# qdrant/qdrant

Measured on AMD Instinct MI355X. Metric: QPS @ recall@10, brute-force, d=768 10M vecs, f32 cosine top-10, higher is better.
Workload: dtype f32 (int8 prefilter + exact f32 re-score)

## Files before the change

### qdrant_amd/csrc/api_core.hip

```cpp
#include "api_internal.hpp"

namespace qmx {

static thread_local std::string g_last_error;
const std::string &last_error_text() { return g_last_error; }

void set_error(const char *fmt, ...) {
    char buf[1024];
    va_list ap;
    va_start(ap, fmt);
    vsnprintf(buf, sizeof(buf), fmt, ap);
    va_end(ap);
    g_last_error = buf;
}

int32_t hip_status(hipError_t e, const char *what, const char *file, int line) {
    set_error("HIP error %d (%s) at %s:%d: %s", (int)e, hipGetErrorString(e), file, line, what);
    (void)hipGetLastError();
    switch (e) {
        case hipErrorOutOfMemory: return QMX_ERR_OUT_OF_MEMORY;
        case hipErrorNoDevice:
        case hipErrorInvalidDevice:
        case hipErrorNoBinaryForGpu:
        case hipErrorInsufficientDriver: return QMX_ERR_NO_DEVICE;
        case hipErrorNotReady: return QMX_ERR_NOT_READY;
        case hipErrorInvalidValue: return QMX_ERR_BAD_ARG;
        default: return QMX_ERR_OTHER;
    }
}

static const char *const g_option_names[OPT_COUNT] = {"no_mfma_scan", "no_mfma16", "no_prescan", "prescan_shift", "hnsw_log_cap", "no_split_scan", "split_min_queries", "no_split256", "no_pq_pair", "no_pq_prefilter", "pq_prefilter_min_queries", "hnsw_pq_per_cu", "tq_rotate_block", "no_topk_small", "verify_max_per_query", "hnsw_pq_direct_walk", "hnsw_pq_table_build", "hnsw_no_pq_prefilter", "hnsw_no_lds_visited", "pq_lut_no_lds", "hnsw_per_cu", "hnsw_reference_heap_order", "tq_wide_min_queries", "tq_wide_high_digit", "sq_wide_min_queries", "i8_resident", "i8_dense_epilogue", "i8_sample_stride", "i8_sample_scan", "i8_sample_rows", "prescan_beside_scan", "group_matrix_bytes", "debug"};
struct OptionTable {
    std::atomic<int64_t> v[OPT_COUNT];
    int64_t initial[OPT_COUNT];
    OptionTable() {
        for (int i = 0; i < OPT_COUNT; ++i) {
            char env[64] = "QMX_";
            size_t k = 4;
            for (const char *c = g_option_names[i]; *c && k + 1 < sizeof(env); ++c) env[k++] = (char)toupper((unsigned char)*c);
            env[k] = 0;
            const char *e = getenv(env);
            int64_t val = 0;
            if (e) { val = (*e >= '0' && *e <= '9') ? atoll(e) : 1; }
            if (i == OPT_PRESCAN_SHIFT && !e) val = 10;
            if (i == OPT_SPLIT_MIN_QUERIES && !e) val = 1;
            if (i == OPT_PQ_PREFILTER_MIN_QUERIES && !e) val = 4;
            if (i == OPT_TQ_WIDE_MIN_QUERIES && !e) val = 33;
            if (i == OPT_SQ_WIDE_MIN_QUERIES && !e) val = 33;
            if (i == OPT_I8_RESIDENT && !e) val = 1;
            if (i == OPT_I8_DENSE_EPILOGUE && !e) val = 1;
            if (i == OPT_I8_SAMPLE_STRIDE && !e) val = 16;
            if (i == OPT_I8_SAMPLE_SCAN && !e) val = 1;
            if (i == OPT_PRESCAN_BESIDE_SCAN && !e) val = 1;
            initial[i] = val;
            v[i].store(val, std::memory_order_relaxed);
        }
    }
};
static OptionTable g_options;
int64_t option(Option o) { return g_options.v[o].load(std::memory_order_relaxed); }

static thread_local const void *g_last_kernel = nullptr;
const void *last_noted_kernel() { return g_last_kernel; }
void note_kernel(const void *host_function) { g_last_kernel = host_function; }

void clear_stale_error() {
    hipError_t e = hipGetLastError();
    if (e != hipSuccess) {
// ... 98 lines not shown
```

### qdrant_amd/csrc/api_search.hip

```cpp
#include "api_internal.hpp"

extern "C" {

struct SearchCall {
    qmx_query *q;
    uint32_t top;
    const uint32_t *d_ids;
    uint64_t n_cand;
    qmx_scored_point *d_out;
    uint32_t *d_counts;
    const volatile uint8_t *is_stopped;
    qmx_counters *counters;
    bool timed;
    uint32_t launches;
};

static ScanArgs tile_args(const qmx_query *q, uint32_t top, uint64_t n_cand, uint32_t tile0, uint32_t nq_tile) {
    ScanArgs a;
    fill_args(q, tile0, nq_tile, a);
    a.n_cand = n_cand;
    a.top = top;
    return a;
}
static ScanArgs tile_args(const SearchCall &c, uint32_t tile0, uint32_t nq_tile) { return tile_args(c.q, c.top, c.n_cand, tile0, nq_tile); }
// ... 170 lines not shown
        ScanArgs a = tile_args(c, 0, nq_sub);
        a.queries = (const char *)q->sp_fq.p + (size_t)p0 * q->q_stride;
        if (fof_packed) a.del.filter_of = fof_packed + p0;
        a.partial = (uint64_t *)q->partial.p;
        a.gthr = gthr_packed + p0;
        a.run_if = run_if;
        const int fqt = (int)std::max<uint32_t>(16, pow2_ceil(nq_sub));
        a.partial_qt = (uint32_t)fqt;
        uint32_t grid = (uint32_t)q->seg->num_cus * 8;
        QMX_TRY(scan(q->stream, fqt, a, q->seg->num_cus, &grid));
        QMX_TRY(launch_merge_keys(q->stream, (const uint64_t *)q->partial.p, grid, (uint32_t)fqt, nq_sub, c.top, c.d_out, c.d_counts, c.top, 0, nullptr, run_if,
                                  ovf_list + p0));
        if (launches) *launches += 2;
    }
    return split_stage(q, "fallback (conditional)");
}

static int32_t pq_overflow_pass(const SearchCall &c, const SplitPlanLayout &pl) {
    qmx_query *q = c.q;
    const qmx_segment *s = q->seg;
    unsigned char *plan = (unsigned char *)q->sp_plan.p;
    uint32_t *ovf_list = (uint32_t *)(plan + pl.list);
    QMX_TRY(launch_split_plan(q->stream, (const uint32_t *)(plan + pl.ovf_q), q->nq, (const uint64_t *)q->gthr.p, ovf_list, (uint64_t *)(plan + pl.gthr_packed),
                              pl.list_cap, (uint32_t *)(plan + pl.count), (int *)(plan + pl.run16), (int *)(plan + pl.run64), pl.n_run64, (SplitStats *)plan, nullptr, 0,
                              nullptr));
    ScanArgs a = tile_args(c, 0, q->nq);
    a.q_map = ovf_list;
    a.run_if = (const int *)(plan + pl.count);
    const uint64_t want = (c.n_cand + 1023) / 1024, cap = std::max<uint64_t>(1, ((uint64_t)s->num_cus * 2 + q->nq - 1) / q->nq);
    uint32_t slabs = (uint32_t)std::max<uint64_t>(1, std::min(want, cap));
// ... 134 lines not shown
    QMX_TRY(verify_and_sort(c, vp, q->nq));
    QMX_TRY(overflow_passes(c, pl, q->nq, TQW_FQT, sq ? overflow_scan_sq : overflow_scan_tq, &c.launches));
    q->last_split = true;
    q->last_pq = false;
    q->last_fqt = TQW_FQT;
    close_counters(c, (uint64_t)q->nq * c.n_cand,
                   (uint64_t)n_tiles * c.n_cand * s->row_bytes + (uint64_t)((q->nq + MAX_QT_MFMA - 1) / MAX_QT_MFMA) * S * s->row_bytes, c.launches, q->nq);
    return QMX_OK;
}

struct SplitTiles {
    SplitPlanLayout pl;
    VerifyPool vp{};
    uint64_t S = 0;
    bool i8_sample = false;
    std::vector<std::pair<uint32_t, uint32_t>> tiles;
    SplitTiles(uint32_t nq, uint32_t fqt) : pl(nq, fqt) {}
};

static inline float split_rel_band(bool half, uint32_t dim) {
    const float acc = (float)dim * 1.1920929e-7f;
    return (half ? 9.765625e-4f + 9.5367432e-7f : 1.9073486e-6f) + acc;
}

static int32_t split_begin(const SearchCall &c, const SearchPlan &plan, SplitTiles &sp) {
    qmx_query *q = c.q;
    const qmx_segment *s = q->seg;
    QMX_TRY(q->sp_bq.reserve(split_query_bytes(s->dim)));
    QMX_TRY(q->sp_f32.reserve(SplitF32::floats * sizeof(float)));
    QMX_TRY(q->sp_cand.reserve((size_t)plan.split_qt * SPLIT_CAND_CAP * sizeof(uint64_t)));
// ... 92 lines not shown
    if (!sp.i8_sample) QMX_TRY(bound_enqueue(c, tile0, nq_tile, (const uint32_t *)q->sp_sample.p, sp.S, c.top, a.del, nullptr, true));
    QMX_TRY(split_stage(q, "prescan"));
    int *tile_ovf = (int *)((unsigned char *)q->sp_plan.p + sp.pl.tile_ovf) + sp.tiles.size();
    if (plan.route == ROUTE_I8_COPY) QMX_TRY(i8_copy_scan(c, sp, a, tile0, nq_tile, tile_ovf));
    else QMX_TRY(f16_split_scan(c, sp, a, tile0, nq_tile, tile_ovf));
    QMX_TRY(split_stage(q, "select"));
    sp.tiles.push_back({tile0, nq_tile});
    return QMX_OK;
}

static int32_t split_finish(const SearchCall &c, const SearchPlan &plan, const SplitTiles &sp) {
    qmx_query *q = c.q;
    const uint32_t first = sp.tiles.front().first, last = sp.tiles.back().first + sp.tiles.back().second;
    QMX_REQUIRE(first == 0, QMX_ERR_OTHER, "split tiles must start at query 0");
    QMX_TRY(verify_and_sort(c, sp.vp, last));
    QMX_TRY(overflow_passes(c, sp.pl, last, plan.split_fqt, overflow_scan_f32, nullptr));
    q->last_split = true;
    q->last_pq = false;
    q->last_fqt = plan.split_fqt;
    return QMX_OK;
}

static int32_t exact_tile(SearchCall &c, const SearchPlan &plan, uint32_t tile0, uint32_t nq_tile) {
    qmx_query *q = c.q;
    const qmx_segment *s = q->seg;
    const int qt = (int)pow2_ceil(nq_tile);
    for (uint32_t pass = 0; pass < plan.n_pass; ++pass) {
        QMX_CHECK_CANCELLED(c.is_stopped);
        const uint32_t off = pass * MAX_TOP_FAST;
        const uint32_t ptop = std::min<uint32_t>(MAX_TOP_FAST, c.top - off);
        ScanArgs a = tile_args(c, tile0, nq_tile);
        a.ids = c.d_ids;
        a.top = ptop;
        a.partial = (uint64_t *)q->partial.p;
// ... 25 lines not shown
    const qmx_segment *s = q->seg;
    if (is_sparse(s)) QMX_REFUSE_FILTERS(q);
    if (is_sparse(s)) return sparse_search_enqueue(q, top, d_ids, n_ids, d_out, d_counts, is_stopped, counters, timed);
    SearchCall c{q, top, d_ids, d_ids ? n_ids : s->scan_rows(), d_out, d_counts, is_stopped, counters, timed, 0};
    const SearchPlan plan = search_plan(q, top, d_ids, c.n_cand);
    q->last_counters = qmx_counters{};
    q->last_split = false;
    if (plan.route == ROUTE_TQ_L1) return tq_l1_search(c, plan);
    if (plan.route == ROUTE_PQ_PREFILTER) return pq_prefilter_search(c);
    if (plan.route == ROUTE_TQ_WIDE || plan.route == ROUTE_SQ_WIDE) return wide_exact_search(c);
    const uint32_t TQ = plan.tile_q;
    QMX_TRY(q->partial.reserve((size_t)s->num_cus * 8 * std::min<uint32_t>(TQ, MAX_QT_TOPK) * std::min<uint32_t>(top, MAX_TOP_FAST) * sizeof(uint64_t)));
    if (plan.n_pass > 1) QMX_TRY(q->bounds.reserve((size_t)TQ * sizeof(uint64_t)));
    QMX_TRY(q->gthr.reserve((size_t)std::max<uint32_t>(q->nq_padded, SPLIT_QT_MAX) * sizeof(uint64_t)));
    SplitTiles sp(q->nq, plan.split_fqt);
    if (plan.split()) QMX_TRY(split_begin(c, plan, sp));
    for (uint32_t tile0 = 0; tile0 < q->nq; tile0 += TQ) {
        const uint32_t nq_tile = std::min<uint32_t>(TQ, q->nq - tile0);
        if (plan.tile_splits(nq_tile)) QMX_TRY(split_tile(c, plan, sp, tile0, nq_tile));
        else QMX_TRY(exact_tile(c, plan, tile0, nq_tile));
    }
    if (!sp.tiles.empty()) QMX_TRY(split_finish(c, plan, sp));
    uint32_t split_q = 0;
    uint64_t bytes = 0;
    for (auto &t : sp.tiles) {
        split_q += t.second;
        bytes += c.n_cand * (uint64_t)s->dim * (s->split_i8 ? 1 : s->d_rows_split && s->split_half ? 2 : 4);
        if (sp.i8_sample) {
            const uint32_t group = split_i8_sample_queries(s->dim, t.second);
            bytes += (uint64_t)((t.second + group - 1) / group) * q->sp_sample_n * s->dim + (uint64_t)t.second * std::min<uint32_t>(top, MAX_TOP_FAST) * s->row_bytes;
// ... 217 lines not shown
```

### qdrant_amd/csrc/common.hpp

```cpp
#pragma once
#include <hip/hip_runtime.h>
#include <hip/hip_fp16.h>
#include <stdint.h>
#include <atomic>
#include <string>

#include "../../include/qdrant_amd.h"

namespace qmx {

void set_error(const char *fmt, ...);
int32_t hip_status(hipError_t e, const char *what, const char *file, int line);
void clear_stale_error();

enum Option {
    OPT_NO_MFMA_SCAN = 0,
    OPT_NO_MFMA16,
    OPT_NO_PRESCAN,
    OPT_PRESCAN_SHIFT,
    OPT_HNSW_LOG_CAP,
    OPT_NO_SPLIT_SCAN,
    OPT_SPLIT_MIN_QUERIES,
    OPT_NO_SPLIT256,
    OPT_NO_PQ_PAIR,
// ... 7 lines not shown
    OPT_HNSW_PQ_TABLE_BUILD,
    OPT_HNSW_NO_PQ_PREFILTER,
    OPT_HNSW_NO_LDS_VISITED,
    OPT_PQ_LUT_NO_LDS,
    OPT_HNSW_PER_CU,
    OPT_HNSW_REFERENCE_HEAP_ORDER,
    OPT_TQ_WIDE_MIN_QUERIES,
    OPT_TQ_WIDE_HIGH_DIGIT,
    OPT_SQ_WIDE_MIN_QUERIES,
    OPT_I8_RESIDENT,
    OPT_I8_DENSE_EPILOGUE,
    OPT_I8_SAMPLE_STRIDE,
    OPT_I8_SAMPLE_SCAN,
    OPT_I8_SAMPLE_ROWS,
    OPT_PRESCAN_BESIDE_SCAN,
    OPT_GROUP_MATRIX_BYTES,
    OPT_DEBUG,
    OPT_COUNT
};
int64_t option(Option o);
struct DeviceOnce {
    std::atomic<uint64_t> done{0};
    int dev = 0;
    bool need() {
        if (hipGetDevice(&dev) != hipSuccess) { dev = 0; return true; }
        return dev >= 64 || !(done.load(std::memory_order_acquire) & (1ull << dev));
    }
    void mark() { if (dev < 64) done.fetch_or(1ull << dev, std::memory_order_release); }
};
void note_kernel(const void *host_function);
// ... 123 lines not shown
```

### qdrant_amd/csrc/kernels.hpp

```cpp
#pragma once
#include "common.hpp"

namespace qmx {

constexpr int MAX_QT = 16;
constexpr int SCAN_BLOCK = 512;
constexpr int MAX_TOP_FAST = 64;

struct TqEc {
    const int16_t *weights;
    const float *xm;
    float weight_scale, mm_const;
};
struct ScanArgs {
    const void *rows;
    uint64_t n_rows;
    uint64_t row_stride;
    uint32_t dim;
    uint32_t nseg;
    uint32_t rem_pieces;
    uint32_t tail_start;
    uint32_t aux_off;
    uint32_t nq;
    const void *queries;
// ... 243 lines not shown
int32_t launch_scan_sq(hipStream_t st, int distance, int qt, ScanMode mode, const ScanArgs &a, int num_cus,
                       uint32_t *grid_out);
int32_t launch_sq_encode(hipStream_t st, int distance, const qmx_sq_params &sp, uint32_t dim, const float *in, uint64_t n,
                         uint8_t *codes_out, uint64_t codes_stride, float *offsets_out, uint8_t *rows_out, int is_query,
                         uint32_t aux_off);
int32_t launch_sq_split(hipStream_t st, const void *rows, uint64_t row_stride, uint64_t n, uint32_t actual_dim, void *codes,
                        float *offsets);
int32_t launch_sq_gather_rows(hipStream_t st, const void *codes, const float *offsets, uint32_t actual_dim, const uint32_t *ids,
                              uint32_t n, uint64_t n_rows, void *rows_out, int *err_flag);
int32_t launch_sq_internal_query(hipStream_t st, const void *codes, const float *offsets, uint32_t actual_dim, const uint32_t *ids,
                                 uint32_t nq, uint64_t n_rows, float shift, void *tile, uint32_t q_stride, uint32_t aux_off,
                                 int *err_flag);
bool mfma16_dim_ok(int qt, uint32_t dim);
bool mfma16_scan_ok(int qt, ScanMode mode, const ScanArgs &a);
int32_t launch_scan_f32_mfma16(hipStream_t st, int qt, const ScanArgs &a, int num_cus, uint32_t *grid_out);
bool split_scan_ok(const ScanArgs &a);
size_t split_query_bytes(uint32_t dim);
float split_row_scale(float row_maxabs);
int32_t launch_split_row_stats(hipStream_t st, const void *rows, uint64_t row_stride, uint64_t n, uint32_t dim, uint32_t *d_stats);
int32_t launch_split_pack_queries(hipStream_t st, const float *d_q, uint32_t nq, uint32_t dim, float *d_qmax, float *d_qnorm, void *d_bq, int half, uint32_t qt);
int32_t launch_split_thresholds(hipStream_t st, const uint64_t *d_gthr, const float *d_qnorm, const float *d_qmax, uint32_t nq, float rel_band, float row_norm_max,
                                float row_scale, float *d_scales, float *d_thr, float *d_band, uint32_t qt, uint32_t *d_cand_cnt, uint32_t n_cnt);
int32_t launch_scan_f32_split(hipStream_t st, const ScanArgs &a, const void *d_bq, float row_scale, const float *d_scales, const float *d_thr,
                              uint64_t *d_cand, uint32_t *d_cand_cnt, uint32_t cap, int num_cus, const void *d_rows_split, int half, void *d_wlists, uint32_t phase, uint32_t qt);
int32_t launch_regroup_lists(hipStream_t st, const DeletedView &del, const void *d_wlist, const uint32_t *d_wcnt, uint32_t wcap, uint32_t n_lists, uint64_t *d_cand,
                             uint32_t *d_cand_cnt, uint32_t cap, int *d_overflow);
size_t pq_rot_bytes(uint64_t n, uint32_t m);
bool pq_prefilter_shape_ok(uint32_t m, uint32_t ncent);
int32_t launch_pq_rotate(hipStream_t st, const void *codes, uint64_t row_stride, uint64_t n, uint32_t m, void *d_out);
size_t pq_prefilter_table_bytes(uint32_t m, uint32_t nq);
// ... 25 lines not shown
int32_t launch_split_select(hipStream_t st, const uint64_t *d_cand, const uint32_t *d_cand_cnt, uint32_t cap, const float *d_band, uint32_t nq, uint32_t top,
                            const VerifyPool &pool, uint32_t q_base, const int *d_tile_overflow, uint32_t *d_ovf_q, SplitStats *d_stats,
                            const float *d_t_exact = nullptr, bool tighten = false);
bool split_i8_dim_ok(uint32_t dim);
size_t split_i8_copy_bytes(uint64_t n, uint32_t dim);
size_t split_i8_query_bytes(uint32_t dim);
uint32_t split_i8_probe();
int32_t launch_split_i8_colstats(hipStream_t st, const void *rows, uint64_t row_stride, uint64_t n, uint32_t dim, uint32_t *d_colmax, float *d_colsq);
float split_i8_choose_scales(const float *colmax, const float *colsq, uint64_t n, uint32_t dim, float *scale);
int32_t launch_split_i8_rowstats(hipStream_t st, const void *rows, uint64_t row_stride, uint64_t n, uint32_t dim, const float *d_scale, uint32_t *d_stats);
int32_t launch_split_i8_copy(hipStream_t st, const void *rows, uint64_t row_stride, uint64_t n, uint32_t dim, const float *d_scale, void *d_out);
int32_t launch_split_i8_pack(hipStream_t st, const float *d_q, uint32_t nq, uint32_t dim, const float *d_scale, const uint64_t *d_gthr, const uint32_t *d_row_stats,
                             float row_norm_max, void *d_bq, float *d_qscale, float *d_band, float *d_thr, float *d_t_exact, uint32_t *d_cand_cnt, uint32_t n_cnt);
int32_t launch_scan_i8copy(hipStream_t st, const ScanArgs &a, const void *d_bq, const float *d_qscale, const float *d_thr, int num_cus, const void *d_rows_i8,
                           void *d_wlists, uint32_t phase);
int32_t launch_split_i8_probe(hipStream_t st, const uint64_t *d_cand, const uint32_t *d_cand_cnt, uint32_t cap, const float *d_band, uint32_t nq, uint32_t top,
                              const int *d_tile_overflow, uint32_t *d_probe_ids, uint32_t *d_probe_cnt);
int32_t launch_split_i8_bound(hipStream_t st, const float *d_scores, uint32_t *d_probe_cnt, uint32_t nq, uint32_t top, const float *d_band, const float *d_qscale,
                              float *d_thr, float *d_t_exact);
uint32_t split_i8_sample_queries(uint32_t dim, uint32_t nq);
int32_t launch_scan_i8copy_sample(hipStream_t st, const void *d_rows_i8, const void *d_bq, uint32_t dim, const uint32_t *d_sample, uint32_t n_tiles, uint32_t nq,
                                  const float *d_qscale, float *d_scores);
int32_t launch_split_i8_picks(hipStream_t st, const qmx_scored_point *d_lists, const uint32_t *d_counts, uint32_t nq, uint32_t top, const float *d_band,
                              uint32_t *d_probe_ids, uint32_t *d_probe_cnt);
int32_t launch_split_i8_sample_bound(hipStream_t st, const float *d_scores, const uint32_t *d_probe_ids, uint32_t *d_probe_cnt, uint32_t nq, uint32_t top,
                                     float *d_band, const float *d_qscale, float *d_thr, float *d_t_exact, uint64_t *d_gthr);
bool tq4w_shape_ok(const ScanArgs &a);
size_t tq4w_query_bytes(uint32_t code_bytes);
size_t tq4w_wlists_counts_bytes(int num_cus);
size_t tq4w_wlists_bytes(int num_cus);
// ... 32 lines not shown
int32_t launch_pairs_pq(hipStream_t st, const ScanArgs &a, const PairSel &sel, uint64_t n_items, int num_cus);
int32_t launch_pq_lut(hipStream_t st, uint32_t distance, uint32_t dim, const qmx_pq_params &pq, const float *d_centroids,
                      const float *d_queries, uint32_t nq, float *d_lut);
int32_t launch_pq_internal(hipStream_t st, uint32_t distance, uint32_t dim, const qmx_pq_params &pq, const float *d_centroids,
                           const float *d_pair, const void *rows, uint64_t row_stride, uint64_t n_rows, const uint32_t *a_ids, const uint32_t *b_ids,
                           uint32_t n, float *out, int *err_flag);
int32_t launch_pq_train(hipStream_t st, uint32_t dim, uint32_t chunk_size, uint32_t n_centroids, const float *d_data, uint64_t n,
                        uint32_t max_iters, float accuracy, uint32_t threads, float *d_centroids, uint32_t *iters_host);
int32_t launch_pq_encode(hipStream_t st, uint32_t dim, const qmx_pq_params &pq, const float *d_centroids, const float *d_in,
                         uint64_t n, uint8_t *d_codes);
int32_t launch_pack_queries(hipStream_t st, int dtype, int distance, const void *src, int src_is_encoded,
                            uint32_t src_stride, uint32_t nq, uint32_t dim, void *tile, uint32_t q_stride, uint32_t aux_off);
int32_t launch_merge_keys(hipStream_t st, const uint64_t *partial, uint32_t n_lists,
                          uint32_t qt_stride, uint32_t nq, uint32_t top, qmx_scored_point *out,
                          uint32_t *out_counts, uint32_t out_stride = 0, uint32_t out_offset = 0,
                          uint64_t *next_bound = nullptr, const int *run_if = nullptr, const uint32_t *out_map = nullptr, uint32_t shared_grid = 0);
int32_t launch_merge_points(hipStream_t st, const qmx_scored_point *lists, const uint32_t *list_counts,
                            const uint32_t *list_idx_base, uint32_t n_lists, uint32_t nq, uint32_t k, qmx_scored_point *out,
                            uint32_t *out_counts, uint64_t list_stride = 0, uint64_t count_stride = 0);
int32_t launch_split_candidates(hipStream_t st, const qmx_scored_point *cand, const uint32_t *cand_cnt, uint32_t n_per, uint32_t nq,
                                uint32_t *ids, uint32_t top, qmx_scored_point *out, uint32_t *out_counts);
int32_t launch_sort_scored(hipStream_t st, const float *scores, const uint32_t *ids, const uint32_t *counts, uint32_t n_per_query, uint32_t nq, uint32_t top,
                           qmx_scored_point *out, uint32_t *out_counts, const uint32_t *offsets = nullptr);

int32_t launch_custom_combine(hipStream_t st, const qmx_custom_query *d_queries, uint32_t n_queries, const float *d_sims, uint64_t n,
                              const float *d_coefs, float *d_out);
int32_t launch_maxsim(hipStream_t st, const float *d_sims, uint64_t n_rows, const uint32_t *d_qfirst, uint32_t n_queries, const uint64_t *d_offsets,
                      uint32_t n_points, const uint32_t *d_ids, uint64_t n, float *d_out, int *err_flag);
int32_t launch_custom_topk(hipStream_t st, const float *d_scores, uint64_t n, const uint32_t *d_ids, const DeletedView &del, uint32_t n_queries,
                           uint32_t top, qmx_scored_point *d_out, uint32_t *d_counts, uint64_t *d_bound = nullptr,
                           bool beside_scan = false);
// ... 212 lines not shown
```

### qdrant_amd/csrc/scan_mfma16.hip

```cpp
#include "scan_common.hpp"

namespace qmx {

typedef float f32x4 __attribute__((ext_vector_type(4)));
typedef __attribute__((address_space(3))) unsigned char lds_byte;

constexpr int M16_ROWP = 1024 + 16;
constexpr int M16_STAGE = 16 * M16_ROWP;

__device__ __forceinline__ void glds16(const unsigned char *row, uint32_t lane_off, uint32_t lds_dst) {
    unsigned keep;
    asm volatile("s_mov_b32 %0, m0\n\ts_mov_b32 m0, %3\n\ts_nop 0\n\tglobal_load_lds_dwordx4 %1, %2 nt\n\ts_mov_b32 m0, %0"
                 : "=&s"(keep) : "v"(lane_off), "s"(row), "s"(lds_dst) : "memory");
}
__device__ __forceinline__ void glds16v(const unsigned char *src, uint32_t lds_dst) {
    unsigned keep;
    asm volatile("s_mov_b32 %0, m0\n\ts_mov_b32 m0, %2\n\ts_nop 0\n\tglobal_load_lds_dwordx4 %1, off nt\n\ts_mov_b32 m0, %0"
                 : "=&s"(keep) : "v"(src), "s"(lds_dst) : "memory");
}
__device__ __forceinline__ uint64_t uniform_u64(uint64_t v) {
    const uint32_t lo = (uint32_t)__builtin_amdgcn_readfirstlane((int)(uint32_t)v), hi = (uint32_t)__builtin_amdgcn_readfirstlane((int)(uint32_t)(v >> 32));
    return ((uint64_t)hi << 32) | lo;
}

// ... 9 lines not shown
    asm volatile("s_load_dwordx2 %0, %1, 0x0\n\ts_waitcnt lgkmcnt(0)" : "=s"(wv) : "s"(p) : "memory");
    return (wv >> (id & 63)) & 1;
}
__device__ __forceinline__ bool live_uniform(const DeletedView &d, uint32_t id, const uint32_t *filter_of, uint64_t stride, uint32_t q) {
    const bool vdel = (d.vec_deleted && id < d.n_vec_bits) ? bit_get_uniform(d.vec_deleted, id) : false;
    const bool pdel = d.point_deleted ? (id < d.n_point_bits ? bit_get_uniform(d.point_deleted, id) : true) : !(id < d.n_rows);
    const uint64_t *allowed = d.allowed;
    if (filter_of) {
        const uint32_t f = sload_u32(filter_of + q);
        allowed = f == QMX_FILTER_NONE ? nullptr : d.allowed + (uint64_t)f * stride;
    }
    const bool ok = allowed ? (id < d.n_allowed_bits && bit_get_uniform(allowed, id)) : true;
    return !vdel && !pdel && ok;
}

template <int NW, int NT, int KPS >
struct M16Shape {
    static constexpr int QT = 16 * NT;
    static constexpr int JW = 8 / NW;
    static constexpr int CW = 4 * JW;
    static constexpr int RPW = 16 / NW;
    static constexpr int STAGE = KPS == 2 ? M16_STAGE : M16_STAGE / 2;
    static constexpr int NBUF = (NW == 4 ? 4 : 7) * (KPS == 2 ? 1 : 2);
    static constexpr int XCH = NW * NT * 4 * 64 * 4;
    static constexpr int IDR = 16 * 16 * 4;
    static constexpr int LDS = NBUF * STAGE + XCH + IDR;
    static constexpr int VPS = KPS == 2 ? RPW : RPW / 2;
    static constexpr int PW = NT * 4 / NW;
    static_assert(PW == 1 || PW == 2, "the NT * 4 planes of a tile are split evenly over the waves");
};

template <int KSTEPS , int NW, int NT, int DBG = 0 ,
          bool LAG = (NW == 8 && NT == 4 && KSTEPS == 6) ,
          bool IDS = false ,
          bool PERQ = false >
__global__ __launch_bounds__(NW * 64, NW == 4 ? 2 : 1) void scan_f32_mfma16_kernel(const ScanArgs a) {
    if (a.run_if && *a.run_if == 0) return;
    constexpr int KPS = KSTEPS % 2 == 0 ? 2 : 1;
    constexpr int KS = KSTEPS / KPS;
    typedef M16Shape<NW, NT, KPS> S;
    constexpr int QT = S::QT, JW = S::JW, CW = S::CW, RPW = S::RPW, NBUF = S::NBUF, PW = S::PW;
    constexpr int M16_STAGE_B = S::STAGE;
    static_assert(!LAG || KPS == 2, "the lagging-wave schedule is written for two-step stages");
    extern __shared__ __attribute__((aligned(16))) unsigned char smem[];
    const int tid = threadIdx.x;
    const int lane = tid & 63;
    const int w = __builtin_amdgcn_readfirstlane(tid >> 6);
    const int n = lane & 15, kk = lane >> 4;
    const bool lag = LAG && (((a.flags & 0x100u) ? (w & 1) : (w >= NW / 2)) != 0);
    const uint32_t lds0 = (uint32_t)(uintptr_t)(lds_byte *)smem;
    const unsigned char *rows = reinterpret_cast<const unsigned char *>(a.rows);
    const int top = (int)a.top;
    auto chain_rel = [](int ci) { return 8 * (ci / JW) + 4 * (ci % JW); };

    float bq[CW][KSTEPS][NT];
// ... 279 lines not shown
            }
        }
        if (lane < top) a.partial[((uint64_t)blockIdx.x * QT + q) * utop + lane] = merged;
    }
}

template <int KSTEPS, int NW, int NT, int DBG = 0, bool LAG = (NW == 8 && NT == 4 && KSTEPS == 6), bool IDS = false>
static int32_t launch_m16(hipStream_t st, const ScanArgs &a, int num_cus, uint32_t *grid_out) {
    if constexpr (!IDS && DBG == 0 && LAG == (NW == 8 && NT == 4 && KSTEPS == 6)) {
        if (a.ids) {
            if constexpr (KSTEPS >= 5 && NW == 4 && NT == 2) return launch_m16<KSTEPS, 8, 2, 0, false, true>(st, a, num_cus, grid_out);
            else return launch_m16<KSTEPS, NW, NT, 0, LAG, true>(st, a, num_cus, grid_out);
        }
    }
    typedef M16Shape<NW, NT, (KSTEPS % 2 == 0 ? 2 : 1)> S;
    auto kfn = a.del.filter_of ? scan_f32_mfma16_kernel<KSTEPS, NW, NT, DBG, LAG, IDS, true> : scan_f32_mfma16_kernel<KSTEPS, NW, NT, DBG, LAG, IDS, false>;
    static thread_local DeviceOnce attr_once;
    if (attr_once.need()) {
        QMX_HIP(hipFuncSetAttribute(reinterpret_cast<const void *>(scan_f32_mfma16_kernel<KSTEPS, NW, NT, DBG, LAG, IDS, false>), hipFuncAttributeMaxDynamicSharedMemorySize,
                                    160 * 1024));
        QMX_HIP(hipFuncSetAttribute(reinterpret_cast<const void *>(scan_f32_mfma16_kernel<KSTEPS, NW, NT, DBG, LAG, IDS, true>), hipFuncAttributeMaxDynamicSharedMemorySize,
                                    160 * 1024));
        attr_once.mark();
    }
    const uint64_t n_tiles = (a.n_cand + 15) / 16;
    int per_cu = 0;
    QMX_HIP(hipOccupancyMaxActiveBlocksPerMultiprocessor(&per_cu, kfn, NW * 64, (size_t)S::LDS));
    if (per_cu < 1) per_cu = 1;
    const uint64_t cap = (uint64_t)num_cus * per_cu;
    uint32_t grid = (uint32_t)(n_tiles < cap ? n_tiles : cap);
    if (grid < 1) grid = 1;
    if (grid_out) {
        if (*grid_out && grid > *grid_out) grid = *grid_out;
        *grid_out = grid;
    }
    ScanArgs b = a;
#ifdef QMX_TUNING
// ... 44 lines not shown
            const char *dbg = getenv("QMX_M16_DBG");
            if (dbg && dbg[0] == '2') return launch_m16<6, 8, 4, 2>(st, a, num_cus, grid_out);
            if (dbg && dbg[0] == '3') return launch_m16<6, 8, 4, 3>(st, a, num_cus, grid_out);
            if (dbg && dbg[0] == '4') return launch_m16<6, 8, 4, 4, false>(st, a, num_cus, grid_out);
            if (dbg && dbg[0] == '6') return launch_m16<6, 8, 4, 6, false>(st, a, num_cus, grid_out);
            if (dbg && dbg[0] == '7') return launch_m16<6, 8, 4, 3, false>(st, a, num_cus, grid_out);
            if (dbg && dbg[0] == '5') return launch_m16<6, 8, 4, 0, false>(st, a, num_cus, grid_out);
        }
#endif
        return launch_m16_steps<8, 4, 1, 6>(st, ksteps, a, num_cus, grid_out);
    }
    set_error("mfma16 scan: unsupported shape");
    return QMX_ERR_BAD_ARG;
}

}
```

### qdrant_amd/csrc/scan_split.hip

```cpp
#include <type_traits>

#include "scan_common.hpp"

namespace qmx {

typedef _Float16 half8 __attribute__((ext_vector_type(8)));
typedef _Float16 half4 __attribute__((ext_vector_type(4)));
typedef float f32x4s __attribute__((ext_vector_type(4)));

constexpr int SP_BM = 256;
constexpr int SP_QT = 128;
constexpr int SP_QT_MAX = 256;
constexpr int SP_THREADS = 768;
constexpr int SP_CONSUMERS = 8;
constexpr int SP_A_UNITS = SP_BM * 2 * 4;
constexpr int SP_B_UNITS = SP_QT * 2 * 4;
constexpr int SP_BRING = 4;
constexpr int SP_LDS = (2 * SP_A_UNITS + SP_BRING * SP_B_UNITS) * 16;

__device__ __forceinline__ uint32_t sp_unit(uint32_t t, uint32_t hl, uint32_t kq, uint32_t m) { return ((t * 2 + hl) * 4 + kq) * 16 + (m ^ (2 * kq)); }

__device__ __forceinline__ void sp_split4(const f32x4s v, float scale, half4 &h, half4 &l) {
#pragma unroll
    for (int i = 0; i < 4; ++i) {
// ... 2010 lines not shown
                              float *d_thr, float *d_t_exact) {
    ::qmx::clear_stale_error();
    hipLaunchKernelGGL(sp_i8_bound_kernel, dim3(nq), dim3(64), 0, st, d_scores, d_probe_cnt, top, d_band, d_qscale, d_thr, d_t_exact);
    QMX_HIP(hipGetLastError());
    return QMX_OK;
}
uint32_t split_i8_sample_queries(uint32_t dim, uint32_t nq) {
    const uint32_t nch = dim / 128;
    if (nch > SP8R_MAX_NCH) return 16;
    const size_t free_lds = (size_t)160 * 1024 - sp8r_lds_bytes(nch);
    uint32_t pick = 16;
    for (uint32_t c = 32; c <= 64; c *= 2)
        if ((size_t)nch * (c / 16) * 2048 <= free_lds && c / 2 < nq) pick = c;
    return pick;
}
int32_t launch_scan_i8copy_sample(hipStream_t st, const void *d_rows_i8, const void *d_bq, uint32_t dim, const uint32_t *d_sample, uint32_t n_tiles, uint32_t nq,
                                  const float *d_qscale, float *d_scores) {
    QMX_REQUIRE(d_rows_i8 && split_i8_dim_ok(dim) && nq >= 1 && nq <= (uint32_t)SP_QT && n_tiles >= 1, QMX_ERR_BAD_ARG, "int8 sample scan of %u queries", nq);
    const uint32_t nch = dim / 128, NQ = split_i8_sample_queries(dim, nq);
    const size_t lds_bytes = (size_t)nch * (NQ / 16) * 2048;
    QMX_REQUIRE(lds_bytes <= 65536, QMX_ERR_OTHER, "int8 sample scan: %zu B of query images", lds_bytes);
    const dim3 grid((n_tiles + 7) / 8, (nq + NQ - 1) / NQ);
    ::qmx::clear_stale_error();
    if (NQ == 64)
        hipLaunchKernelGGL(scan_i8copy_sample_kernel<64>, grid, dim3(256), lds_bytes, st, (const uint4 *)d_rows_i8, (const uint4 *)d_bq, nch, d_sample, n_tiles, nq, d_qscale, d_scores);
    else if (NQ == 32)
        hipLaunchKernelGGL(scan_i8copy_sample_kernel<32>, grid, dim3(256), lds_bytes, st, (const uint4 *)d_rows_i8, (const uint4 *)d_bq, nch, d_sample, n_tiles, nq, d_qscale, d_scores);
    else
        hipLaunchKernelGGL(scan_i8copy_sample_kernel<16>, grid, dim3(256), lds_bytes, st, (const uint4 *)d_rows_i8, (const uint4 *)d_bq, nch, d_sample, n_tiles, nq, d_qscale, d_scores);
    QMX_HIP(hipGetLastError());
// ... 19 lines not shown
```

### qdrant_amd/csrc/topk_merge.hip

```cpp
#include "kernels.hpp"

namespace qmx {

constexpr int MERGE_BLOCK = 256;
constexpr int MERGE_NW = MERGE_BLOCK / WAVE;

__device__ __forceinline__ uint64_t block_finish(uint64_t list, int top, uint32_t q, qmx_scored_point *out, uint32_t out_stride,
                                                 uint32_t out_offset, uint32_t *out_counts) {
    __shared__ uint64_t sh[MERGE_NW][WAVE];
    __shared__ uint64_t sh_bound;
    const int lane = threadIdx.x & 63, wave = threadIdx.x >> 6;
    __syncthreads();
    sh[wave][lane] = list;
    __syncthreads();
    if (wave == 0) {
        uint64_t merged = sh[0][lane];
        for (int w = 1; w < MERGE_NW; ++w) wave_offer(merged, sh[w][lane], top, lane);
        const bool ok = lane < top && merged != 0;
        if (lane < top) {
            qmx_scored_point p;
            p.idx = ok ? key_idx(merged) : 0u;
            p.score = ok ? key_score(merged) : 0.0f;
            out[(uint64_t)q * out_stride + out_offset + lane] = p;
        }
        const uint32_t cnt = (uint32_t)__popcll(__ballot(ok));
        const uint64_t last = readlane_u64(merged, top - 1);
        if (lane == 0) {
            out_counts[q] = (out_offset ? out_counts[q] : 0u) + cnt;
            sh_bound = cnt == (uint32_t)top ? last : 0ull;
        }
    }
    __syncthreads();
    return sh_bound;
}

__global__ __launch_bounds__(MERGE_BLOCK) void merge_keys_kernel(const uint64_t *partial, uint32_t n_lists,
                                                                 uint32_t qt_stride, uint32_t top,
                                                                 qmx_scored_point *out, uint32_t *out_counts, uint32_t out_stride,
                                                                 uint32_t out_offset, uint64_t *next_bound, const int *run_if, const uint32_t *out_map,
                                                                 uint32_t shared_grid) {
    if (run_if && *run_if == 0) return;
    const uint32_t q = blockIdx.x;
    if (shared_grid) {
        const uint32_t cnt = (uint32_t)*run_if, nq_eff = cnt < gridDim.x ? cnt : gridDim.x;
        n_lists = shared_grid / nq_eff;
        qt_stride = nq_eff;
    }
    const uint32_t oq = out_map ? out_map[q] : q;
    if (oq == 0xFFFFFFFFu) return;
    const int lane = threadIdx.x & 63, wave = threadIdx.x >> 6;
    uint64_t list = 0;
    for (uint32_t l = wave; l < n_lists; l += MERGE_NW) {
        const uint64_t key = lane < (int)top ? partial[((uint64_t)l * qt_stride + q) * top + lane] : 0;
        wave_offer(list, key, (int)top, lane);
    }
    const uint64_t nb = block_finish(list, (int)top, oq, out, out_stride, out_offset, out_counts);
    if (next_bound && threadIdx.x == 0) next_bound[q] = nb;
}

__global__ __launch_bounds__(MERGE_BLOCK) void merge_points_kernel(const qmx_scored_point *lists,
                                                                   const uint32_t *list_counts,
                                                                   const uint32_t *list_idx_base, uint32_t n_lists,
                                                                   uint32_t nq, uint32_t k, qmx_scored_point *out,
                                                                   uint32_t *out_counts, uint64_t list_stride, uint64_t count_stride) {
    extern __shared__ uint32_t seen_ids[];
    const uint32_t q = blockIdx.x;
    const int lane = threadIdx.x & 63, wave = threadIdx.x >> 6;
    const uint32_t total = n_lists * k;
// ... 48 lines not shown
            const uint32_t i = base + lane;
            uint64_t key = i < cnt ? make_key(scores[first + i], ids[first + i]) : 0;
            if (key >= bound) key = 0;
            wave_offer(list, key, ptop, lane);
        }
        bound = block_finish(list, ptop, q, out, top, off, out_counts);
        if (bound == 0) {
            for (uint32_t i = off + WAVE + threadIdx.x; i < top; i += MERGE_BLOCK) out[(uint64_t)q * top + i] = qmx_scored_point{0u, 0.0f};
            break;
        }
    }
}

int32_t launch_merge_keys(hipStream_t st, const uint64_t *partial, uint32_t n_lists, uint32_t qt_stride,
                          uint32_t nq, uint32_t top, qmx_scored_point *out, uint32_t *out_counts, uint32_t out_stride,
                          uint32_t out_offset, uint64_t *next_bound, const int *run_if, const uint32_t *out_map, uint32_t shared_grid) {
    if (nq == 0) return QMX_OK;
    if (out_stride == 0) out_stride = top;
    ::qmx::clear_stale_error();
    hipLaunchKernelGGL(merge_keys_kernel, dim3(nq), dim3(MERGE_BLOCK), 0, st, partial, n_lists, qt_stride, top, out, out_counts,
                       out_stride, out_offset, next_bound, run_if, out_map, shared_grid);
    QMX_HIP(hipGetLastError());
    return QMX_OK;
}
int32_t launch_merge_points(hipStream_t st, const qmx_scored_point *lists, const uint32_t *list_counts,
                            const uint32_t *list_idx_base, uint32_t n_lists, uint32_t nq, uint32_t k,
                            qmx_scored_point *out, uint32_t *out_counts, uint64_t list_stride, uint64_t count_stride) {
    if (nq == 0) return QMX_OK;
    if (list_stride == 0) list_stride = (uint64_t)nq * k;
    if (count_stride == 0) count_stride = nq;
    QMX_REQUIRE((uint64_t)n_lists * k * sizeof(uint32_t) <= 64 * 1024, QMX_ERR_NOT_SUPPORTED,
                "merge of %u lists x %u entries exceeds the 64 KiB seen-id table", n_lists, k);
    ::qmx::clear_stale_error();
    hipLaunchKernelGGL(merge_points_kernel, dim3(nq), dim3(MERGE_BLOCK), (size_t)n_lists * k * sizeof(uint32_t), st, lists, list_counts, list_idx_base, n_lists, nq, k, out, out_counts,
                       list_stride, count_stride);
    QMX_HIP(hipGetLastError());
// ... 73 lines not shown
```

Before: 100,400.

## Run split overflow fallback as one grouped MFMA16 launch beside the int8 scan

Adds a grouped MFMA16 f32 scan kernel that covers every 16-query overflow group in a single 2D launch with a smaller three-stage LDS ring, plus a grouped merge_keys mode. On the int8-copy route it replaces the per-tile conditional fallback passes, so the fallback can co-reside with the int8 scan on each CU. It only turns on when LDS and register footprints of both kernels fit together. The costs are a larger partial-list buffer and a shallower prefetch ring, which may slow the fallback kernel itself.

```diff
diff --git a/qdrant_amd/csrc/api_core.hip b/qdrant_amd/csrc/api_core.hip
--- a/qdrant_amd/csrc/api_core.hip
+++ b/qdrant_amd/csrc/api_core.hip
@@ -29,7 +29,7 @@
     }
 }
 
-static const char *const g_option_names[OPT_COUNT] = {"no_mfma_scan", "no_mfma16", "no_prescan", "prescan_shift", "hnsw_log_cap", "no_split_scan", "split_min_queries", "no_split256", "no_pq_pair", "no_pq_prefilter", "pq_prefilter_min_queries", "hnsw_pq_per_cu", "tq_rotate_block", "no_topk_small", "verify_max_per_query", "hnsw_pq_direct_walk", "hnsw_pq_table_build", "hnsw_no_pq_prefilter", "hnsw_no_lds_visited", "pq_lut_no_lds", "hnsw_per_cu", "hnsw_reference_heap_order", "tq_wide_min_queries", "tq_wide_high_digit", "sq_wide_min_queries", "i8_resident", "i8_dense_epilogue", "i8_sample_stride", "i8_sample_scan", "i8_sample_rows", "prescan_beside_scan", "group_matrix_bytes", "debug"};
+static const char *const g_option_names[OPT_COUNT] = {"no_mfma_scan", "no_mfma16", "no_prescan", "prescan_shift", "hnsw_log_cap", "no_split_scan", "split_min_queries", "no_split256", "no_pq_pair", "no_pq_prefilter", "pq_prefilter_min_queries", "hnsw_pq_per_cu", "tq_rotate_block", "no_topk_small", "verify_max_per_query", "hnsw_pq_direct_walk", "hnsw_pq_table_build", "hnsw_no_pq_prefilter", "hnsw_no_lds_visited", "pq_lut_no_lds", "hnsw_per_cu", "hnsw_reference_heap_order", "tq_wide_min_queries", "tq_wide_high_digit", "sq_wide_min_queries", "i8_resident", "i8_dense_epilogue", "i8_sample_stride", "i8_sample_scan", "i8_sample_rows", "prescan_beside_scan", "fallback_beside_scan", "group_matrix_bytes", "debug"};
 struct OptionTable {
     std::atomic<int64_t> v[OPT_COUNT];
     int64_t initial[OPT_COUNT];
@@ -52,6 +52,7 @@
             if (i == OPT_I8_SAMPLE_STRIDE && !e) val = 16;
             if (i == OPT_I8_SAMPLE_SCAN && !e) val = 1;
             if (i == OPT_PRESCAN_BESIDE_SCAN && !e) val = 1;
+            if (i == OPT_FALLBACK_BESIDE_SCAN && !e) val = 1;
             initial[i] = val;
             v[i].store(val, std::memory_order_relaxed);
         }
diff --git a/qdrant_amd/csrc/api_search.hip b/qdrant_amd/csrc/api_search.hip
--- a/qdrant_amd/csrc/api_search.hip
+++ b/qdrant_amd/csrc/api_search.hip
@@ -208,6 +208,51 @@
         if (launches) *launches += 2;
     }
     return split_stage(q, "fallback (conditional)");
+}
+
+static int32_t fallback_groups_fit(const qmx_query *q, uint32_t top, bool *fit) {
+    const qmx_segment *s = q->seg;
+    *fit = false;
+    if (option(OPT_FALLBACK_BESIDE_SCAN) <= 0 || !mfma16_dim_ok(16, s->dim) || top > 64 || s->row_stride % 16 != 0) return QMX_OK;
+    const uint32_t ks = s->dim / 128, perq = q->has_filters ? 1 : 0, res = option(OPT_I8_RESIDENT) > 0 ? 1 : 0;
+    static std::atomic<int> known[2][2][17];
+    int k = known[res][perq][ks].load(std::memory_order_relaxed);
+    if (k == 0) {
+        size_t scan_lds = 0, pass_lds = 0;
+        int scan_regs = 0, pass_regs = 0;
+        QMX_TRY(split_i8_scan_footprint(s->dim, &scan_lds, &scan_regs));
+        QMX_TRY(mfma16_groups_footprint(s->dim, perq != 0, &pass_lds, &pass_regs));
+        k = scan_lds + pass_lds <= (size_t)160 * 1024 && scan_regs + pass_regs <= 512 ? 1 : 2;
+        known[res][perq][ks].store(k, std::memory_order_relaxed);
+    }
+    *fit = k == 1;
+    return QMX_OK;
+}
+static size_t overflow_groups_partial_bytes(const qmx_query *q, uint32_t top) {
+    return (size_t)q->seg->num_cus * 2 * ((q->nq + 15) / 16) * 16 * top * sizeof(uint64_t);
+}
+static int32_t overflow_groups_pass(const SearchCall &c, const SplitPlanLayout &pl, uint32_t nq) {
+    qmx_query *q = c.q;
+    unsigned char *plan = (unsigned char *)q->sp_plan.p;
+    uint32_t *ovf_list = (uint32_t *)(plan + pl.list);
+    uint64_t *gthr_packed = (uint64_t *)(plan + pl.gthr_packed);
+    if (q->has_filters) QMX_TRY(q->filter_of_packed.reserve((size_t)pl.list_cap * 4));
+    QMX_TRY(launch_split_plan(q->stream, (const uint32_t *)(plan + pl.ovf_q), nq, (const uint64_t *)q->gthr.p, ovf_list, gthr_packed, pl.list_cap,
+                              (uint32_t *)(plan + pl.count), (int *)(plan + pl.run16), (int *)(plan + pl.run64), pl.n_run64, (SplitStats *)plan, q->d_queries,
+                              q->q_stride, q->sp_fq.p, q->has_filters ? (const uint32_t *)q->filter_of.p : nullptr, (uint32_t *)q->filter_of_packed.p));
+    ScanArgs a = tile_args(c, 0, nq);
+    a.queries = q->sp_fq.p;
+    if (q->has_filters) a.del.filter_of = (const uint32_t *)q->filter_of_packed.p;
+    a.partial = (uint64_t *)q->partial.p;
+    a.partial_qt = 16;
+    a.gthr = gthr_packed;
+    a.run_if = (const int *)(plan + pl.count);
+    QMX_REQUIRE(mfma16_scan_ok(16, SCAN_TOPK, a), QMX_ERR_OTHER, "split fallback shape");
+    uint32_t grid = (uint32_t)q->seg->num_cus * 2;
+    QMX_REQUIRE(nq <= q->nq && overflow_groups_partial_bytes(q, c.top) <= q->partial.cap, QMX_ERR_OTHER, "split fallback: partial lists");
+    QMX_TRY(launch_scan_f32_mfma16_groups(q->stream, a, q->seg->num_cus, &grid));
+    QMX_TRY(launch_merge_keys(q->stream, (const uint64_t *)q->partial.p, grid, 16, nq, c.top, c.d_out, c.d_counts, c.top, 0, nullptr, a.run_if, ovf_list, 0, true));
+    return split_stage(q, "fallback (conditional, one launch)");
 }
 
 static int32_t pq_overflow_pass(const SearchCall &c, const SplitPlanLayout &pl) {
@@ -372,6 +417,7 @@
     VerifyPool vp{};
     uint64_t S = 0;
     bool i8_sample = false;
+    bool ovf_groups = false;
     std::vector<std::pair<uint32_t, uint32_t>> tiles;
     SplitTiles(uint32_t nq, uint32_t fqt) : pl(nq, fqt) {}
 };
@@ -494,10 +540,11 @@
     const uint32_t first = sp.tiles.front().first, last = sp.tiles.back().first + sp.tiles.back().second;
     QMX_REQUIRE(first == 0, QMX_ERR_OTHER, "split tiles must start at query 0");
     QMX_TRY(verify_and_sort(c, sp.vp, last));
-    QMX_TRY(overflow_passes(c, sp.pl, last, plan.split_fqt, overflow_scan_f32, nullptr));
+    if (sp.ovf_groups) QMX_TRY(overflow_groups_pass(c, sp.pl, last));
+    else QMX_TRY(overflow_passes(c, sp.pl, last, plan.split_fqt, overflow_scan_f32, nullptr));
     q->last_split = true;
     q->last_pq = false;
-    q->last_fqt = plan.split_fqt;
+    q->last_fqt = sp.ovf_groups ? 16 : plan.split_fqt;
     return QMX_OK;
 }
 
@@ -553,6 +600,10 @@
     if (plan.n_pass > 1) QMX_TRY(q->bounds.reserve((size_t)TQ * sizeof(uint64_t)));
     QMX_TRY(q->gthr.reserve((size_t)std::max<uint32_t>(q->nq_padded, SPLIT_QT_MAX) * sizeof(uint64_t)));
     SplitTiles sp(q->nq, plan.split_fqt);
+    if (plan.route == ROUTE_I8_COPY) {
+        QMX_TRY(fallback_groups_fit(q, top, &sp.ovf_groups));
+        if (sp.ovf_groups) QMX_TRY(q->partial.reserve(overflow_groups_partial_bytes(q, top)));
+    }
     if (plan.split()) QMX_TRY(split_begin(c, plan, sp));
     for (uint32_t tile0 = 0; tile0 < q->nq; tile0 += TQ) {
         const uint32_t nq_tile = std::min<uint32_t>(TQ, q->nq - tile0);
diff --git a/qdrant_amd/csrc/common.hpp b/qdrant_amd/csrc/common.hpp
--- a/qdrant_amd/csrc/common.hpp
+++ b/qdrant_amd/csrc/common.hpp
@@ -45,6 +45,7 @@
     OPT_I8_SAMPLE_SCAN,
     OPT_I8_SAMPLE_ROWS,
     OPT_PRESCAN_BESIDE_SCAN,
+    OPT_FALLBACK_BESIDE_SCAN,
     OPT_GROUP_MATRIX_BYTES,
     OPT_DEBUG,
     OPT_COUNT
diff --git a/qdrant_amd/csrc/kernels.hpp b/qdrant_amd/csrc/kernels.hpp
--- a/qdrant_amd/csrc/kernels.hpp
+++ b/qdrant_amd/csrc/kernels.hpp
@@ -281,6 +281,8 @@
 bool mfma16_dim_ok(int qt, uint32_t dim);
 bool mfma16_scan_ok(int qt, ScanMode mode, const ScanArgs &a);
 int32_t launch_scan_f32_mfma16(hipStream_t st, int qt, const ScanArgs &a, int num_cus, uint32_t *grid_out);
+int32_t launch_scan_f32_mfma16_groups(hipStream_t st, const ScanArgs &a, int num_cus, uint32_t *grid_out);
+int32_t mfma16_groups_footprint(uint32_t dim, bool perq, size_t *lds_bytes, int *regs_per_simd);
 bool split_scan_ok(const ScanArgs &a);
 size_t split_query_bytes(uint32_t dim);
 float split_row_scale(float row_maxabs);
@@ -336,6 +338,7 @@
                              float row_norm_max, void *d_bq, float *d_qscale, float *d_band, float *d_thr, float *d_t_exact, uint32_t *d_cand_cnt, uint32_t n_cnt);
 int32_t launch_scan_i8copy(hipStream_t st, const ScanArgs &a, const void *d_bq, const float *d_qscale, const float *d_thr, int num_cus, const void *d_rows_i8,
                            void *d_wlists, uint32_t phase);
+int32_t split_i8_scan_footprint(uint32_t dim, size_t *lds_bytes, int *regs_per_simd);
 int32_t launch_split_i8_probe(hipStream_t st, const uint64_t *d_cand, const uint32_t *d_cand_cnt, uint32_t cap, const float *d_band, uint32_t nq, uint32_t top,
                               const int *d_tile_overflow, uint32_t *d_probe_ids, uint32_t *d_probe_cnt);
 int32_t launch_split_i8_bound(hipStream_t st, const float *d_scores, uint32_t *d_probe_cnt, uint32_t nq, uint32_t top, const float *d_band, const float *d_qscale,
@@ -398,7 +401,8 @@
 int32_t launch_merge_keys(hipStream_t st, const uint64_t *partial, uint32_t n_lists,
                           uint32_t qt_stride, uint32_t nq, uint32_t top, qmx_scored_point *out,
                           uint32_t *out_counts, uint32_t out_stride = 0, uint32_t out_offset = 0,
-                          uint64_t *next_bound = nullptr, const int *run_if = nullptr, const uint32_t *out_map = nullptr, uint32_t shared_grid = 0);
+                          uint64_t *next_bound = nullptr, const int *run_if = nullptr, const uint32_t *out_map = nullptr, uint32_t shared_grid = 0,
+                          bool grouped = false);
 int32_t launch_merge_points(hipStream_t st, const qmx_scored_point *lists, const uint32_t *list_counts,
                             const uint32_t *list_idx_base, uint32_t n_lists, uint32_t nq, uint32_t k, qmx_scored_point *out,
                             uint32_t *out_counts, uint64_t list_stride = 0, uint64_t count_stride = 0);
diff --git a/qdrant_amd/csrc/scan_mfma16.hip b/qdrant_amd/csrc/scan_mfma16.hip
--- a/qdrant_amd/csrc/scan_mfma16.hip
+++ b/qdrant_amd/csrc/scan_mfma16.hip
@@ -47,14 +47,16 @@
     return !vdel && !pdel && ok;
 }
 
-template <int NW, int NT, int KPS >
+template <int NW, int NT, int KPS ,
+          int RING = 0 >
 struct M16Shape {
     static constexpr int QT = 16 * NT;
     static constexpr int JW = 8 / NW;
     static constexpr int CW = 4 * JW;
     static constexpr int RPW = 16 / NW;
     static constexpr int STAGE = KPS == 2 ? M16_STAGE : M16_STAGE / 2;
-    static constexpr int NBUF = (NW == 4 ? 4 : 7) * (KPS == 2 ? 1 : 2);
+    static constexpr int NBUF = (RING ? RING : NW == 4 ? 4 : 7) * (KPS == 2 ? 1 : 2);
+    static_assert(NBUF >= 3, "the stage loop keeps one stage in registers, one landing and at least one in flight");
     static constexpr int XCH = NW * NT * 4 * 64 * 4;
     static constexpr int IDR = 16 * 16 * 4;
     static constexpr int LDS = NBUF * STAGE + XCH + IDR;
@@ -66,12 +68,26 @@
 template <int KSTEPS , int NW, int NT, int DBG = 0 ,
           bool LAG = (NW == 8 && NT == 4 && KSTEPS == 6) ,
           bool IDS = false ,
+          int RING = 0 ,
+          bool GROUPS = false ,
           bool PERQ = false >
-__global__ __launch_bounds__(NW * 64, NW == 4 ? 2 : 1) void scan_f32_mfma16_kernel(const ScanArgs a) {
-    if (a.run_if && *a.run_if == 0) return;
+__global__ __launch_bounds__(NW * 64, NW == 4 ? 2 : 1) void scan_f32_mfma16_kernel(const ScanArgs a_launch) {
+    ScanArgs a = a_launch;
+    if constexpr (GROUPS) {
+        static_assert(NT == 1, "a block row serves one 16-query tile");
+        const uint32_t q0 = 16u * blockIdx.y;
+        if (q0 >= (uint32_t)*a.run_if) return;
+        a.queries = reinterpret_cast<const char *>(a.queries) + (size_t)q0 * a.q_stride;
+        a.gthr += q0;
+        if constexpr (PERQ) a.del.filter_of += q0;
+        a.partial += (uint64_t)blockIdx.y * gridDim.x * 16u * a.top;
+        a.nq = a.nq - q0 < 16u ? a.nq - q0 : 16u;
+    } else {
+        if (a.run_if && *a.run_if == 0) return;
+    }
     constexpr int KPS = KSTEPS % 2 == 0 ? 2 : 1;
     constexpr int KS = KSTEPS / KPS;
-    typedef M16Shape<NW, NT, KPS> S;
+    typedef M16Shape<NW, NT, KPS, RING> S;
     constexpr int QT = S::QT, JW = S::JW, CW = S::CW, RPW = S::RPW, NBUF = S::NBUF, PW = S::PW;
     constexpr int M16_STAGE_B = S::STAGE;
     static_assert(!LAG || KPS == 2, "the lagging-wave schedule is written for two-step stages");
@@ -381,13 +397,13 @@
         }
     }
     typedef M16Shape<NW, NT, (KSTEPS % 2 == 0 ? 2 : 1)> S;
-    auto kfn = a.del.filter_of ? scan_f32_mfma16_kernel<KSTEPS, NW, NT, DBG, LAG, IDS, true> : scan_f32_mfma16_kernel<KSTEPS, NW, NT, DBG, LAG, IDS, false>;
+    auto kfn = a.del.filter_of ? scan_f32_mfma16_kernel<KSTEPS, NW, NT, DBG, LAG, IDS, 0, false, true> : scan_f32_mfma16_kernel<KSTEPS, NW, NT, DBG, LAG, IDS, 0, false, false>;
     static thread_local DeviceOnce attr_once;
     if (attr_once.need()) {
-        QMX_HIP(hipFuncSetAttribute(reinterpret_cast<const void *>(scan_f32_mfma16_kernel<KSTEPS, NW, NT, DBG, LAG, IDS, false>), hipFuncAttributeMaxDynamicSharedMemorySize,
-                                    160 * 1024));
-        QMX_HIP(hipFuncSetAttribute(reinterpret_cast<const void *>(scan_f32_mfma16_kernel<KSTEPS, NW, NT, DBG, LAG, IDS, true>), hipFuncAttributeMaxDynamicSharedMemorySize,
-                                    160 * 1024));
+        QMX_HIP(hipFuncSetAttribute(reinterpret_cast<const void *>(scan_f32_mfma16_kernel<KSTEPS, NW, NT, DBG, LAG, IDS, 0, false, false>),
+                                    hipFuncAttributeMaxDynamicSharedMemorySize, 160 * 1024));
+        QMX_HIP(hipFuncSetAttribute(reinterpret_cast<const void *>(scan_f32_mfma16_kernel<KSTEPS, NW, NT, DBG, LAG, IDS, 0, false, true>),
+                                    hipFuncAttributeMaxDynamicSharedMemorySize, 160 * 1024));
         attr_once.mark();
     }
     const uint64_t n_tiles = (a.n_cand + 15) / 16;
@@ -462,4 +478,52 @@
     return QMX_ERR_BAD_ARG;
 }
 
-}
+constexpr int M16_GROUPS_RING = 3;
+typedef void (*M16Kernel)(const ScanArgs);
+template <int K0, int K1>
+static M16Kernel m16_groups_kernel(int ksteps, bool perq) {
+    if constexpr (K0 <= K1) {
+        if constexpr (!(K0 > 12 && K0 % 2 == 1)) {
+            if (ksteps == K0)
+                return perq ? scan_f32_mfma16_kernel<K0, 4, 1, 0, false, false, M16_GROUPS_RING, true, true>
+                            : scan_f32_mfma16_kernel<K0, 4, 1, 0, false, false, M16_GROUPS_RING, true, false>;
+        }
+        return m16_groups_kernel<K0 + 1, K1>(ksteps, perq);
+    } else {
+        return nullptr;
+    }
+}
+
+int32_t mfma16_groups_footprint(uint32_t dim, bool perq, size_t *lds_bytes, int *regs_per_simd) {
+    const M16Kernel kfn = mfma16_dim_ok(16, dim) ? m16_groups_kernel<1, 16>((int)(dim / 128), perq) : nullptr;
+    QMX_REQUIRE(kfn != nullptr, QMX_ERR_BAD_ARG, "mfma16 scan: no 16-query shape for rows of %u coordinates", dim);
+    hipFuncAttributes fa;
+    QMX_HIP(hipFuncGetAttributes(&fa, reinterpret_cast<const void *>(kfn)));
+    *lds_bytes = (size_t)M16Shape<4, 1, 2, M16_GROUPS_RING>::LDS + fa.sharedSizeBytes;
+    *regs_per_simd = (fa.numRegs + 7) / 8 * 8;
+    return QMX_OK;
+}
+
+int32_t launch_scan_f32_mfma16_groups(hipStream_t st, const ScanArgs &a, int num_cus, uint32_t *grid_out) {
+    typedef M16Shape<4, 1, 2, M16_GROUPS_RING> S;
+    static_assert(S::LDS == M16Shape<4, 1, 1, M16_GROUPS_RING>::LDS && S::LDS == 55040, "three stages or six half stages");
+    QMX_REQUIRE(a.run_if && a.gthr && a.partial && !a.ids && !a.key_bound && a.nq >= 1 && grid_out, QMX_ERR_BAD_ARG, "mfma16 groups: a packed conditional pass");
+    const bool perq = a.del.filter_of != nullptr;
+    const M16Kernel kfn = m16_groups_kernel<1, 16>((int)(a.nseg / 4), perq);
+    QMX_REQUIRE(kfn != nullptr, QMX_ERR_BAD_ARG, "mfma16 scan: unsupported row length");
+    const uint64_t n_tiles = (a.n_cand + 15) / 16;
+    int per_cu = 0;
+    QMX_HIP(hipOccupancyMaxActiveBlocksPerMultiprocessor(&per_cu, kfn, 256, (size_t)S::LDS));
+    if (per_cu < 1) per_cu = 1;
+    const uint64_t cap = (uint64_t)num_cus * per_cu;
+    uint32_t grid = (uint32_t)(n_tiles < cap ? n_tiles : cap);
+    if (grid < 1) grid = 1;
+    if (*grid_out && grid > *grid_out) grid = *grid_out;
+    *grid_out = grid;
+    ::qmx::clear_stale_error();
+    hipLaunchKernelGGL(kfn, dim3(grid, (a.nq + 15) / 16), dim3(256), (size_t)S::LDS, st, a);
+    QMX_HIP(hipGetLastError());
+    return QMX_OK;
+}
+
+}
diff --git a/qdrant_amd/csrc/scan_split.hip b/qdrant_amd/csrc/scan_split.hip
--- a/qdrant_amd/csrc/scan_split.hip
+++ b/qdrant_amd/csrc/scan_split.hip
@@ -2048,6 +2048,16 @@
         if ((size_t)nch * (c / 16) * 2048 <= free_lds && c / 2 < nq) pick = c;
     return pick;
 }
+int32_t split_i8_scan_footprint(uint32_t dim, size_t *lds_bytes, int *regs_per_simd) {
+    const uint32_t nch = dim / 128;
+    const bool resident = option(OPT_I8_RESIDENT) > 0 && nch <= SP8R_MAX_NCH;
+    void (*kfn)(const ScanArgs, const SplitArgs) = resident ? scan_i8copy_kernel_res<1> : scan_i8copy_kernel;
+    hipFuncAttributes fa;
+    QMX_HIP(hipFuncGetAttributes(&fa, reinterpret_cast<const void *>(kfn)));
+    *lds_bytes = (resident ? sp8r_lds_bytes(nch) : (size_t)SP8_LDS) + fa.sharedSizeBytes;
+    *regs_per_simd = SP3_THREADS / 256 * ((fa.numRegs + 7) / 8 * 8);
+    return QMX_OK;
+}
 int32_t launch_scan_i8copy_sample(hipStream_t st, const void *d_rows_i8, const void *d_bq, uint32_t dim, const uint32_t *d_sample, uint32_t n_tiles, uint32_t nq,
                                   const float *d_qscale, float *d_scores) {
     QMX_REQUIRE(d_rows_i8 && split_i8_dim_ok(dim) && nq >= 1 && nq <= (uint32_t)SP_QT && n_tiles >= 1, QMX_ERR_BAD_ARG, "int8 sample scan of %u queries", nq);
diff --git a/qdrant_amd/csrc/topk_merge.hip b/qdrant_amd/csrc/topk_merge.hip
--- a/qdrant_amd/csrc/topk_merge.hip
+++ b/qdrant_amd/csrc/topk_merge.hip
@@ -38,9 +38,16 @@
                                                                  uint32_t qt_stride, uint32_t top,
                                                                  qmx_scored_point *out, uint32_t *out_counts, uint32_t out_stride,
                                                                  uint32_t out_offset, uint64_t *next_bound, const int *run_if, const uint32_t *out_map,
-                                                                 uint32_t shared_grid) {
+                                                                 uint32_t shared_grid, uint32_t grouped) {
     if (run_if && *run_if == 0) return;
     const uint32_t q = blockIdx.x;
+    uint32_t col = q;
+    if (grouped) {
+        if (q >= (uint32_t)*run_if) return;
+        partial += (uint64_t)(q / 16) * n_lists * 16 * top;
+        col = q & 15;
+        qt_stride = 16;
+    }
     if (shared_grid) {
         const uint32_t cnt = (uint32_t)*run_if, nq_eff = cnt < gridDim.x ? cnt : gridDim.x;
         n_lists = shared_grid / nq_eff;
@@ -51,7 +58,7 @@
     const int lane = threadIdx.x & 63, wave = threadIdx.x >> 6;
     uint64_t list = 0;
     for (uint32_t l = wave; l < n_lists; l += MERGE_NW) {
-        const uint64_t key = lane < (int)top ? partial[((uint64_t)l * qt_stride + q) * top + lane] : 0;
+        const uint64_t key = lane < (int)top ? partial[((uint64_t)l * qt_stride + col) * top + lane] : 0;
         wave_offer(list, key, (int)top, lane);
     }
     const uint64_t nb = block_finish(list, (int)top, oq, out, out_stride, out_offset, out_counts);
@@ -130,12 +137,12 @@
 
 int32_t launch_merge_keys(hipStream_t st, const uint64_t *partial, uint32_t n_lists, uint32_t qt_stride,
                           uint32_t nq, uint32_t top, qmx_scored_point *out, uint32_t *out_counts, uint32_t out_stride,
-                          uint32_t out_offset, uint64_t *next_bound, const int *run_if, const uint32_t *out_map, uint32_t shared_grid) {
+                          uint32_t out_offset, uint64_t *next_bound, const int *run_if, const uint32_t *out_map, uint32_t shared_grid, bool grouped) {
     if (nq == 0) return QMX_OK;
     if (out_stride == 0) out_stride = top;
     ::qmx::clear_stale_error();
     hipLaunchKernelGGL(merge_keys_kernel, dim3(nq), dim3(MERGE_BLOCK), 0, st, partial, n_lists, qt_stride, top, out, out_counts,
-                       out_stride, out_offset, next_bound, run_if, out_map, shared_grid);
+                       out_stride, out_offset, next_bound, run_if, out_map, shared_grid, grouped ? 1u : 0u);
     QMX_HIP(hipGetLastError());
     return QMX_OK;
 }
```

New measurement: 103,000, median of 6. 2.6% higher.
